# ultravideo/kvazaar

Measured on AMD Instinct MI355X. Metric: CTUs/s (all-intra ultrafast hot path), higher is better.
Workload: dtype u8/i16 (f64 RD costs)

## Files before the change

### kvazaar_amd/csrc/kvz_ctu.hpp

```cpp
#pragma once
#include <type_traits>
#include "../../include/kvz_hip_types.h"
#include "kvz_ops.hpp"
#include "kvz_rdoq.hpp"
#include "kvz_recon.hpp"
#include "kvz_residual.hpp"
#include "kvz_select.hpp"

namespace kvz {

#define KVZ_CTU_THREADS 128
#ifdef KVZ_HOSTSIM
#define KVZ_FOR_THREADS(tid) for (int tid = 0; tid < KVZ_CTU_THREADS; ++tid)
#ifdef KVZ_HOSTSIM_COUNT_SYNCS
static unsigned long long g_kvz_syncs;
#define KVZ_SYNC() (++g_kvz_syncs)
#else
#define KVZ_SYNC()
#endif
#define KVZ_LDS_ADD(p, v) (*(p) += (v))
#else
#define KVZ_FOR_THREADS(tid) for (int tid = (threadIdx.x + lane_rot) & (KVZ_CTU_THREADS - 1), once_ = 1; once_; once_ = 0)
#define KVZ_SYNC() __syncthreads()
#define KVZ_LDS_ADD(p, v) atomicAdd((p), (v))
// ... 27 lines not shown
{
#ifdef KVZ_HOSTSIM
  *dst += v;
#else
  const int x = row16_sum((int)v);
  const u32 total = (u32)(__builtin_amdgcn_readlane(x, 15) + __builtin_amdgcn_readlane(x, 31) + __builtin_amdgcn_readlane(x, 47) + __builtin_amdgcn_readlane(x, 63));
  if ((threadIdx.x & 63) == 0 && total) atomicAdd(dst, total);
#endif
}

#define KVZ_MREF_STRIDE 36
#define KVZ_MREF_ORG 16
#define KVZ_MREF32_STRIDE 68
#define KVZ_MREF32_ORG 32

#ifdef KVZ_HOSTSIM
struct Pk16 { i16 lo, hi; };
KVZ_DEV Pk16 pk_make(int lo, int hi) { Pk16 r = { (i16)lo, (i16)hi }; return r; }
KVZ_DEV Pk16 pk_add(Pk16 a, Pk16 b) { return pk_make(a.lo + b.lo, a.hi + b.hi); }
KVZ_DEV Pk16 pk_sub(Pk16 a, Pk16 b) { return pk_make(a.lo - b.lo, a.hi - b.hi); }
KVZ_DEV u32 pk_absmax(Pk16 a) { return (u32)imax(iabs(a.lo), iabs(a.hi)); }
#else
typedef short Pk16 __attribute__((ext_vector_type(2)));
KVZ_DEV Pk16 pk_make(int lo, int hi) { Pk16 r; r.x = (short)lo; r.y = (short)hi; return r; }
KVZ_DEV Pk16 pk_add(Pk16 a, Pk16 b) { return a + b; }
KVZ_DEV Pk16 pk_sub(Pk16 a, Pk16 b) { return a - b; }
KVZ_DEV u32 pk_absmax(Pk16 a)
{
  const Pk16 m = __builtin_elementwise_max(a, -a);
  return (u32)imax((int)m.x, (int)m.y);
}
KVZ_DEV u32 pk_abs2_biased(Pk16 a, u32 acc)
{
  unsigned x;
  __builtin_memcpy(&x, &a, 4);
  const unsigned t = __builtin_amdgcn_alignbit(x, x, 16);
  Pk16 sw, r;
  __builtin_memcpy(&sw, &t, 4);
  r = a * pk_make(1, -1) + sw;
  unsigned rr;
  __builtin_memcpy(&rr, &r, 4);
  return __builtin_amdgcn_sad_u16(rr, 0x80008000u, acc);
}
#define KVZ_PK_BIAS pk_make(-32768, 0)
#endif

#ifndef KVZ_HOSTSIM
}
#include "kvz_mfma.hpp"
namespace kvz {
#endif

#define KVZ_PROF_PU_AT (2 * KVZ_P_COUNT + 16)
#define KVZ_PROF_WORDS (4 * KVZ_P_COUNT + 16)
enum { KVZ_P_INIT = 0, KVZ_P_REFS, KVZ_P_PRED35, KVZ_P_SATD, KVZ_P_SELECT, KVZ_P_RPRED, KVZ_P_FDCT, KVZ_P_QUANT, KVZ_P_IDCT, KVZ_P_RECON,
       KVZ_P_COST, KVZ_P_COPY, KVZ_P_FINISH, KVZ_P_MISC, KVZ_P_COEFFBITS, KVZ_P_RDOQ, KVZ_P_COUNT };
#if defined(KVZ_CTU_PROFILE) && !defined(KVZ_HOSTSIM)
#define KVZ_PROF(cat) prof_mark(cat)
#define KVZ_PROF_SYNC(cat) do { KVZ_SYNC(); prof_mark(cat); } while (0)
#else
#define KVZ_PROF(cat)
#define KVZ_PROF_SYNC(cat)
#endif

KVZ_DEV u8 load_shared_byte(const u8 *p)
{
#ifdef KVZ_HOSTSIM
  return *p;
#else
  const unsigned long long a = (unsigned long long)p;
  const unsigned w = __hip_atomic_load((const unsigned *)(a & ~3ull), __ATOMIC_RELAXED, __HIP_MEMORY_SCOPE_AGENT);
  return (u8)(w >> (8 * (a & 3)));
#endif
}
KVZ_DEV u32 load_shared_dword(const u8 *p)
{
#ifdef KVZ_HOSTSIM
  u32 w;
  __builtin_memcpy(&w, p, 4);
  return w;
#else
  return __hip_atomic_load((const unsigned *)p, __ATOMIC_RELAXED, __HIP_MEMORY_SCOPE_AGENT);
#endif
}

#ifdef KVZ_HOSTSIM
#define KVZ_ALIGNED(p, n) (p)
#define KVZ_ROLLED
#else
#define KVZ_ALIGNED(p, n) __builtin_assume_aligned((p), (n))
#define KVZ_ROLLED _Pragma("nounroll")
#endif
KVZ_DEV int mover_lane(int tid)
{
#ifndef KVZ_HOSTSIM
  asm volatile("" : "+v"(tid));
#endif
  return tid;
}
template <int N> struct alignas(N) WideBytes { u32 w[N / 4]; };
template <int N> KVZ_DEV WideBytes<N> wide_load(const void *src)
{
  WideBytes<N> v;
  __builtin_memcpy(&v, KVZ_ALIGNED(src, N), N);
  return v;
}
template <int N> KVZ_DEV void wide_store(void *dst, const WideBytes<N> &v) { __builtin_memcpy(KVZ_ALIGNED(dst, N), &v, N); }
// ... 5 lines not shown
  return v;
}

struct CtuCu { u8 type : 1, depth : 2, tr_depth : 3; u8 mode; uint16_t cbf; };

enum { KVZ_CX_SPLIT = KVZ_HIP_CX_SPLIT, KVZ_CX_PART = KVZ_HIP_CX_PART, KVZ_CX_INTRA = KVZ_HIP_CX_INTRA, KVZ_CX_CHROMA = KVZ_HIP_CX_CHROMA,
       KVZ_CX_CBF_LUMA = KVZ_HIP_CX_CBF_LUMA, KVZ_CX_CBF_CHROMA = KVZ_HIP_CX_CBF_CHROMA, KVZ_CX_SYNTAX_COUNT = KVZ_HIP_CX_SIG_CG, KVZ_CX_COUNT = KVZ_HIP_CX_COUNT };
template <bool CABAC> struct CtxSetT { alignas(4) u8 s[CABAC ? 148 : 12]; };

struct CtuModel {
  double lambda, lambda_sqrt;
  uint64_t coeff_weights;
  int qp;
  u8 adaptive, coeff_cabac, no_wpp, search_32x32, rdoq, search_nxn;
  u8 signhide;
  const float *entropy_fbits;
  const u8 *ctx_init;
};
KVZ_HD void ctu_model_from(const kvz_hip_intra_cost_model *src, CtuModel *dst)
{
  dst->lambda = src->lambda; dst->lambda_sqrt = src->lambda_sqrt; dst->coeff_weights = src->coeff_weights; dst->qp = src->qp; dst->adaptive = src->adaptive != 0;
  dst->coeff_cabac = src->coeff_cabac != 0; dst->no_wpp = src->no_wpp != 0; dst->search_32x32 = src->search_32x32 != 0; dst->rdoq = src->rdoq != 0; dst->search_nxn = src->search_nxn != 0;
  dst->signhide = src->signhide != 0;
  dst->entropy_fbits = src->entropy_fbits;
  dst->ctx_init = src->ctx_init;
}
struct CtuModelTable {
  const CtuModel *models = nullptr;
  const uint16_t *model_of_picture = nullptr;
};
KVZ_HD const CtuModel *picture_model(const CtuModelTable &t, long picture) { return t.models + picture_model(t.model_of_picture, picture); }

struct CtuFrames {
  int W, H, wc, hc;
  long frame_px;
  const u8 *src;
  u8 *rec;
  i16 *coeff;
  i16 *coeff_scratch;
  u8 *cu_depth, *cu_mode;
  u8 *cu_part = nullptr;
  u8 *cu_mode4 = nullptr;
  double *ctu_cost;
  unsigned long long *prof;
  u8 *border;
};
#define KVZ_BORDER_BYTES 512

template <bool CABAC> struct CtuSharedT {
  alignas(16) u8 org[1536];
  alignas(16) u8 dec[6144];
#if defined(KVZ_CTU_PROFILE) && !defined(KVZ_HOSTSIM)
  unsigned long long prof_rq[16];
  unsigned long long prof_acc[64];
  int prof_pu;
#endif
  CtuCu cu[4][64];
  u8 ref[3][2][68];
  u8 fref[2][68];
  union {
    struct {
      alignas(16) i16 tb_big[1536];
      alignas(16) u8 c1[1536];
    };
    struct {
      alignas(16) i16 tb_small[2 * 384];
      alignas(8) u8 org_t[256];
      alignas(16) u8 c2[384];
      alignas(16) i16 lv3_coeff[384];
      u8 mref[15][KVZ_MREF_STRIDE];
      u32 satd_raw[35][4];
    };
  };
  alignas(16) i16 lv2_coeff[384];
  alignas(16) i16 lv1_coeff[1536];
#ifdef KVZ_HOSTSIM
  alignas(16) i16 dct32[32 * 32];
#else
  alignas(16) i16 dct_small[64 + 16];
#endif
  u32 acc[16];
  int8_t preds[3];
  int best_mode;
  double cost[4], split_cost[4];
  double res[4];
  double child_bits[4];
  u32 child_acc[4][9];
  int cbf_any;
  u8 bpx_left[3][66];
  u8 bpx_top[3][98];
  uint16_t nb_cu[2][8];
  u8 dcval[3];
  int8_t mode_disp[35];
  int16_t mode_inv[35];
  QuantScalars qs[4][2];
  double mode_bits_cost[3];
  CtxSetT<CABAC> cab, pre[3], post2;
  float entropy_fbits[128];
  u8 ctx_lps[64];
};

using CtuShared = CtuSharedT<true>;
static_assert(__builtin_offsetof(CtuSharedT<true>, fref) == __builtin_offsetof(CtuSharedT<true>, ref) + 408 && __builtin_offsetof(CtuSharedT<false>, fref) == __builtin_offsetof(CtuSharedT<false>, ref) + 408,
              "Tables::mref_tab addresses the filtered references 408 bytes behind the unfiltered ones");
static_assert(KVZ_MREF_STRIDE == kMrefStride && KVZ_MREF_ORG == kMrefOrg && sizeof(((CtuSharedT<true> *)0)->ref[0][0]) == kMrefRefRow && kMrefFiltered == 408,
              "Tables::mref_tab (kvz_tables.hpp) is built for this layout of the reference arrays");
static_assert(KVZ_CTU_THREADS == 128, "two wavefronts per CTU: thread 64 is 'the other wavefront' (recon_cu8, eval_pu, wide_task, rdoq_unit, prices_coeffs, kHookThread), a 16x16 CU's "
                                      "128 (mode, block) pairs are one round of rough_search, plane_sums routes DPP rows per wavefront, and mref_pre[4] covers Tables::mref_tab's 510 entries");

KVZ_HD int plane_off(int c) { return c ? 3072 + (c << 10) : 0; }

struct RdoqLds {
  i32 ptab[2 * 148];
  u8 diag8[64];
  u8 mode4[4][64][4];
  u8 nb_mode4_left[16];
  u8 c4[96];
  alignas(8) i16 lv4_coeff[96];
  u8 pu_mode[4], pu_cbf[4];
  int pu_cbf_c[2];
  int a3x, a3y, n_pu;
  double split_cost3;
  CtxSetT<true> pre3, post3;
};
template <bool CABAC, bool S32 = false, bool RDOQ = false, bool SH = false, bool LISTS = false> struct CtuProgramT {
  static_assert(!(SH && RDOQ), "kvz_rdoq's own sign hiding is not built");
  static_assert(!(LISTS && (RDOQ || SH)), "scaling lists with kvz_rdoq or sign data hiding are not built");
  using CtxSet = CtxSetT<CABAC>;
  const CtuModel *m;
  const Tables *tb;
  CtuFrames F;
  CtuSharedT<CABAC> *s;
  RdoqLds *rl = nullptr;
  const u32 *lf_y = nullptr, *lf_c = nullptr;
  KVZ_DEV ListFactor factor_at(int c, int l2, int e) const { return list_factor(((c ? lf_c : lf_y) + c * KVZ_LIST_PLANE)[list_index(l2, e)]); }
  static constexpr bool NXN = RDOQ;
  KVZ_DEV bool nxn_on() const { return NXN && m->search_nxn; }
  KVZ_DEV bool cabac_on() const { return CABAC && m->coeff_cabac; }
  KVZ_DEV bool hide_on() const { return SH && m->signhide; }
  int frame, cx, cy;
  int a1x, a1y, a2x, a2y;
  static constexpr int kHookThread = 64;
  int a3q = 0;
  int lane_rot = 0;
#if defined(KVZ_CTU_PROFILE) && !defined(KVZ_HOSTSIM)
  unsigned long long t_last;
  __device__ void prof_mark(int cat)
  {
    if (threadIdx.x == 0) {
      const unsigned long long t = __builtin_amdgcn_s_memtime();
      const int at = s->prof_pu ? 32 : 0;
      s->prof_acc[at + cat] += t - t_last;
      s->prof_acc[at + KVZ_P_COUNT + cat] += 1;
      t_last = __builtin_amdgcn_s_memtime();
    }
  }
#endif

  KVZ_DEV static int uni(int v)
  {
#ifdef KVZ_HOSTSIM
    return v;
#else
    return __builtin_amdgcn_readfirstlane(v);
#endif
  }
  KVZ_DEV const u8 *frame_rec(int c) const { return F.rec + (long)frame * F.frame_px + (c == 0 ? 0 : c == 1 ? (long)F.W * F.H : (long)F.W * F.H * 5 / 4); }
  KVZ_DEV const u8 *frame_src(int c) const { return F.src + (long)frame * F.frame_px + (c == 0 ? 0 : c == 1 ? (long)F.W * F.H : (long)F.W * F.H * 5 / 4); }
  KVZ_DEV int ctu_index() const { return (cy >> 6) * F.wc + (cx >> 6); }
  KVZ_DEV i16 *coeff_level(int level) const
  {
    const long ci = (long)frame * F.wc * F.hc + ctu_index();
    return level == 3 ? F.coeff + ci * 6144 : F.coeff_scratch + ci * 6144;
  }
  struct CandView {
    u8 *buf;
    int bias[3], lw[3];
    KVZ_DEV u8 &at(int c, int x, int y) const { return buf[(c == 0 ? bias[0] : (c == 1 ? bias[1] : bias[2])) + (y << (c == 0 ? lw[0] : lw[1])) + x]; }
  };
  KVZ_DEV CandView cand_view(int lv) const
  {
    CandView v;
    if (NXN && lv == 4) {
      v.buf = rl->c4;
      v.lw[0] = 3; v.lw[1] = v.lw[2] = 2;
      v.bias[0] = -(rl->a3y * 8 + rl->a3x);
      v.bias[1] = 64 - ((rl->a3y >> 1) * 4 + (rl->a3x >> 1));
      v.bias[2] = v.bias[1] + 16;
    } else if (lv == 0 || lv == 3) {
      v.buf = s->dec;
      v.lw[0] = 6; v.lw[1] = v.lw[2] = 5;
      v.bias[0] = 0; v.bias[1] = 4096; v.bias[2] = 5120;
    } else if (lv == 1) {
      v.buf = s->c1;
      v.lw[0] = 5; v.lw[1] = v.lw[2] = 4;
      v.bias[0] = -(a1y * 32 + a1x);
      v.bias[1] = 1024 - ((a1y >> 1) * 16 + (a1x >> 1));
      v.bias[2] = v.bias[1] + 256;
    } else {
      v.buf = s->c2;
      v.lw[0] = 4; v.lw[1] = v.lw[2] = 3;
      v.bias[0] = -(a2y * 16 + a2x);
      v.bias[1] = 256 - ((a2y >> 1) * 8 + (a2x >> 1));
      v.bias[2] = v.bias[1] + 64;
// ... 980 lines not shown
        const u32 v = angular_block_satd<true>(log2w, mode, bx, by, xl, yl, t & 1);
        if (!(t & 1)) s->satd_raw[mode][b] = v;
      }
      {
        const int t = KVZ_CTU_THREADS - 1 - tid;
        if (t < 24 * nblk) {
          const int mb = t >> 3, mi = mb >> lb, mode = mi == 0 ? 34 : mi - 1, b = mb & (nblk - 1), bx = (b & ((w >> 3) - 1)) * 8, by = (b >> (log2w - 3)) * 8;
          const u32 v = flat_block_satd8(log2w, mode, bx, by, xl, yl, tid);
          if ((tid & 7) == 0) s->satd_raw[mode][b] = v;
        }
      }
#endif
    }
    }
    KVZ_SYNC();
    KVZ_PROF(KVZ_P_SATD);
    KVZ_FOR_THREADS(tid) {
      const int final_mode = replay_selection(tid, log2w, nblk);
      if (final_mode >= 0) {
        if (tid == 0) s->best_mode = final_mode;
#ifdef KVZ_HOSTSIM
        const int holders = 1;
#else
        const int holders = 64;
#endif
        for (int i = tid; i < (w >> 3) * (w >> 3); i += holders) {
          const int cell = ((yl >> 3) + (i >> (log2w - 3))) * 8 + (xl >> 3) + (i & ((w >> 3) - 1));
          CtuCu *cu = &s->cu[lv][cell];
          cu->type = 1; cu->depth = (u8)depth; cu->mode = (u8)final_mode; cu->tr_depth = (u8)depth;
          set_mode4(lv, cell, final_mode);
        }
      }
    }
    KVZ_SYNC();
    KVZ_PROF(KVZ_P_SELECT);
  }

  struct TuSet { int x, y, lw , lc ; };
  KVZ_DEV static int tu_log2(const TuSet &t, int c) { return c ? t.lc : t.lw; }
  KVZ_DEV i16 *tbuf(const TuSet &t, int p, int c) const
  {
    if (t.lw == 5) return s->tb_big + (c == 0 ? 0 : (c == 1 ? 1024 : 1280));
    return s->tb_small + p * 384 + (c == 0 ? 0 : (c == 1 ? 256 : 320));
  }
  KVZ_DEV int dct_at(int l2, int k, int i) const
  {
#ifdef KVZ_HOSTSIM
    return s->dct32[(k << (10 - l2)) + i];
#else
    return s->dct_small[(l2 == 3 ? 0 : 64) + (k << l2) + i];
#endif
  }

  KVZ_DEV void transform_big(int l2, i16 *x, bool inverse, int tid, int c) const
  {
#ifndef KVZ_HOSTSIM
    if ((tid >> 6) != (c & 1)) return;
    if (l2 == 5) mfma_transform_block<32>(x, x, inverse, tb, tid & 63);
    else mfma_transform_block<16>(x, x, inverse, tb, tid & 63);
#else
    if (tid != 0) return;
    const int n = 1 << l2;
    i16 tmp[32 * 32];
    for (int pass = 0; pass < 2; pass++) {
      const i16 *src = pass == 0 ? x : tmp;
      i16 *dst = pass == 0 ? tmp : x;
      const int shift = inverse ? (pass == 0 ? 7 : 12) : (pass == 0 ? l2 - 1 : l2 + 6);
      for (int e = 0; e < n * n; e++) {
        const int hi = e >> l2, lo = e & (n - 1);
        dst[e] = inverse ? inv_point(n, [&](int k) { return dct_at(l2, k, lo); }, src, hi, n, shift) : fwd_point(n, [&](int i) { return dct_at(l2, hi, i); }, src, lo << l2, shift);
      }
    }
#endif
  }

  enum RowPlan { ROWS_CU8, ROWS_W16, ROWS_W32_Y, ROWS_W32_C };
  KVZ_DEV u32 plane_sums(RowPlan plan, int tid, int c, u32 v, bool packed, int base) const
  {
#ifdef KVZ_HOSTSIM
    (void)tid;
    if (c < 0) return 0;
    if (packed && plan != ROWS_CU8) { s->acc[3 + c] += v & 0xffffffu; s->acc[6 + c] += v >> 24; }
    else s->acc[base + c] += v;
    return 0;
#else
    (void)c;
    if ((plan == ROWS_W16 || plan == ROWS_W32_C) && tid >= 64) return 0;
    const int x = row16_sum((int)v);
    const u32 r0 = (u32)__builtin_amdgcn_readlane(x, 15), r1 = (u32)__builtin_amdgcn_readlane(x, 31), r2 = (u32)__builtin_amdgcn_readlane(x, 47), r3 = (u32)__builtin_amdgcn_readlane(x, 63);
    if (plan == ROWS_CU8) {
      const u32 luma = r0 + r1 + r2 + r3;
      if ((tid & 63) == 0) {
        if (tid < 64) s->acc[base] += luma;
        else { s->acc[base + 1] += r0; s->acc[base + 2] += r1; }
      }
      return tid < 64 ? luma : (tid < 80 ? r0 : r1);
    }
    if ((tid & 63) != 0) return 0;
    auto put = [&](int plane, u32 a, u32 b) {
      if (packed) {
        const u32 ws = (a & 0xffffffu) + (b & 0xffffffu), n = (a >> 24) + (b >> 24);
        if (n) { atomicAdd(&s->acc[3 + plane], ws); atomicAdd(&s->acc[6 + plane], n); }
        else if (ws) atomicAdd(&s->acc[3 + plane], ws);
      } else if (a + b) atomicAdd(&s->acc[base + plane], a + b);
    };
    if (plan == ROWS_W16) { put(0, r0, r1); put(1, r2, 0); put(2, r3, 0); }
    else if (plan == ROWS_W32_Y) { put(0, r0, r1); put(0, r2, r3); }
    else { put(1, r0, r1); put(2, r2, r3); }
    return 0;
#endif
  }
  KVZ_DEV void finish_planes(int lv, int xl, int yl, int depth, int c0, int c1, bool packed) const
  {
    for (int c = c0; c < c1; c++) {
      u32 n = s->acc[6 + c];
      if (packed) { const u32 pk = s->acc[3 + c]; n = pk >> 24; s->acc[3 + c] = pk & 0xffffffu; s->acc[6 + c] = n; }
      if (NXN && lv == 4) { if (c == 0) rl->pu_cbf[rl->n_pu] = n != 0; else rl->pu_cbf_c[c - 1] = n != 0; }
      else {
        CtuCu *cu = &s->cu[lv][(yl >> 3) * 8 + (xl >> 3)];
        cbf_clear(&cu->cbf, depth, c);
        if (n) cbf_set(&cu->cbf, depth, c);
      }
    }
  }
  KVZ_DEV void hide_signs(int tid, int log2y, int log2c, int scan, const i16 *cf_y, i16 *lv_y, const i16 *cf_u, i16 *lv_u, const i16 *cf_v, i16 *lv_v) const
  {
    if constexpr (SH) {
      const int wv = tid >> 6, lane = tid & 63;
      const int c = wv == 0 ? 0 : 1 + (lane >> 4), i = wv == 0 ? lane : (lane & 15), l2 = wv == 0 ? log2y : log2c, groups = 1 << (2 * l2 - 4);
      const bool live = c < 3 && i < groups;
      const i16 *cf = c == 0 ? cf_y : (c == 1 ? cf_u : cf_v);
      i16 *lv = c == 0 ? lv_y : (c == 1 ? lv_u : lv_v);
      auto group_base = [&](int gi) { const int g = scan_group(l2, scan, gi, diag8()); return (((g >> (l2 - 2)) * 4) << l2) + (g & ((1 << (l2 - 2)) - 1)) * 4; };
      auto group_any = [&](int base) {
        unsigned long long acc4 = 0;
        for (int r = 0; r < 4; r++) { unsigned long long four; __builtin_memcpy(&four, lv + base + (r << l2), 8); acc4 |= four; }
        return acc4 != 0;
      };
      const int base = live ? group_base(i) : 0;
      const bool any = live && group_any(base);
#ifdef KVZ_HOSTSIM
      bool first_visited = true;
      for (int j = i + 1; live && j < groups; j++) first_visited = first_visited && !group_any(group_base(j));
#else
      unsigned long long behind = __ballot(any);
      if (wv != 0) behind = (behind >> (16 * ((c - 1) & 1))) & 0xffffull;
      const bool first_visited = ((behind >> i) >> 1) == 0;
#endif
      if (any) {
// ... 157 lines not shown
    *seg = 0;
    if (lw == 4) {
      if (tid < 32) { *seg = tid; return 0; }
      if (tid >= 64 || (tid & 15) >= 8) return -1;
      *seg = tid & 7;
      return tid < 48 ? 1 : 2;
    }
    if (trip == 0) { *seg = tid; return 0; }
    if (tid >= 64) return -1;
    *seg = tid & 31;
    return 1 + (tid >> 5);
  }
  KVZ_DEV void predict_row8(int l2, int mode, int c, int px0, int py, u8 out[8]) const
  {
    const int w = 1 << l2;
    const bool edges = c == 0 && w < 32;
    const u8 *top = s->ref[c][0], *left = s->ref[c][1];
    if (c == 0 && luma_reads_filtered(l2, mode)) { top = s->fref[0]; left = s->fref[1]; }
    if (mode == 0) {
      const int l = left[py + 1], tr = top[w + 1], bl = left[w + 1];
      const int hb = (w - 1) * l + tr + (py + 1) * bl + w, dl = tr - l, wy = w - 1 - py;
      for (int k = 0; k < 8; k++) out[k] = (u8)(((px0 + k) * dl + top[px0 + k + 1] * wy + hb) >> (l2 + 1));
    } else if (mode == 1) {
      const int dc = s->dcval[c];
      for (int k = 0; k < 8; k++) out[k] = (u8)dc;
      if (edges) {
        if (py == 0) for (int k = 0; k < 8; k++) out[k] = (u8)((top[px0 + k + 1] + 3 * dc + 2) >> 2);
        if (px0 == 0) out[0] = (u8)(py == 0 ? (left[1] + 2 * dc + top[1] + 2) >> 2 : (left[py + 1] + 3 * dc + 2) >> 2);
      }
    } else {
      const int disp = s->mode_disp[mode], inv = s->mode_inv[mode];
      const bool vertical = mode >= 18;
      const u8 *main_ref = vertical ? top : left, *side_ref = vertical ? left : top;
      if (vertical) {
        const int delta = (py + 1) * disp, di = delta >> 5, df = delta & 31;
        int r[9];
        if (disp >= 0) for (int j = 0; j < 9; j++) r[j] = main_ref[px0 + di + j + 1];
        else for (int j = 0; j < 9; j++) r[j] = angular_ref(main_ref, side_ref, px0 + di + j, inv);
        for (int k = 0; k < 8; k++) out[k] = (u8)(((32 - df) * r[k] + df * r[k + 1] + 16) >> 5);
        if (edges && mode == 26 && px0 == 0) out[0] = (u8)iclip(0, 255, (int)out[0] + ((left[py + 1] - left[0]) >> 1));
      } else {
        for (int k = 0; k < 8; k++) {
          const int delta = (px0 + k + 1) * disp, di = delta >> 5, df = delta & 31;
          const int r1 = disp >= 0 ? (int)main_ref[py + di + 1] : angular_ref(main_ref, side_ref, py + di, inv);
          const int r2 = disp >= 0 ? (int)main_ref[py + di + 2] : angular_ref(main_ref, side_ref, py + di + 1, inv);
          int v = ((32 - df) * r1 + df * r2 + 16) >> 5;
          if (edges && mode == 10 && py == 0) v = iclip(0, 255, v + ((top[px0 + k + 1] - top[0]) >> 1));
          out[k] = (u8)v;
        }
      }
    }
  }

  KVZ_DEV void recon_tus(int lv, const TuSet &t, int depth, int mode, bool refs_ready = false)
  {
    const int xl = t.x - cx, yl = t.y - cy;
    const CandView cv = cand_view(lv);
    const bool wide = t.lw >= 4;
    if (!refs_ready) build_refs(lv, t.x, t.y, t.lw, t.lc, true, true);
    if (!RDOQ && t.lw == 3) { recon_cu8(lv, t, depth, mode); return; }
#if defined(KVZ_CTU_PROFILE) && !defined(KVZ_HOSTSIM)
    struct InLarge { CtuSharedT<CABAC> *s; bool on; __device__ InLarge(CtuSharedT<CABAC> *s_, bool on_) : s(s_), on(on_) { if (on && threadIdx.x == 0) s->prof_pu = 1; } __device__ ~InLarge() { if (on && threadIdx.x == 0) s->prof_pu = 0; } } in_large(s, !NXN && t.lw >= 4);
#endif
    if (wide) {
      const int umode = uni(mode);
      KVZ_FOR_THREADS(tid) {
        if (tid < 16) s->acc[tid] = 0;
        for (int trip = 0; trip < wide_trips(t.lw); trip++) {
          int seg;
          const int c = wide_task(t.lw, trip, mover_lane(tid), &seg);
          if (c < 0) continue;
          const int l2 = tu_log2(t, c), sh = c ? 1 : 0, py = seg >> (l2 - 3), px0 = (seg << 3) & ((1 << l2) - 1);
          u8 p[8], o[8];
          i16 res[8];
          predict_row8(l2, umode, c, px0, py, p);
          __builtin_memcpy(o, KVZ_ALIGNED(org_at(c, (xl >> sh) + px0, (yl >> sh) + py), 8), 8);
          for (int k = 0; k < 8; k++) res[k] = (i16)((int)o[k] - (int)p[k]);
          __builtin_memcpy(KVZ_ALIGNED(&cv.at(c, (xl >> sh) + px0, (yl >> sh) + py), 8), p, 8);
          __builtin_memcpy(KVZ_ALIGNED(tbuf(t, 0, c) + (seg << 3), 16), res, 16);
        }
      }
    } else
    KVZ_FOR_THREADS(tid) {
      if (tid < 16) s->acc[tid] = 0;
      for (int c = 0; c < 3; c++) {
        const int l2 = tu_log2(t, c), w = 1 << l2, sh = c ? 1 : 0;
        for (int e = tid; e < w * w; e += KVZ_CTU_THREADS) {
          const int px = e & (w - 1), py = e >> l2;
          const u8 p = predict_pixel(l2, mode, c, px, py);
          cv.at(c, (xl >> sh) + px, (yl >> sh) + py) = p;
          tbuf(t, 0, c)[e] = (i16)((int)*org_at(c, (xl >> sh) + px, (yl >> sh) + py) - (int)p);
        }
      }
    }
    KVZ_SYNC();
    KVZ_PROF(KVZ_P_RPRED);
    for (int pass = 0; pass < 2; pass++) {
      KVZ_FOR_THREADS(tid) {
        for (int c = 0; c < 3; c++) {
          const int l2 = tu_log2(t, c), n = 1 << l2;
          const i16 *src = tbuf(t, pass, c);
          i16 *dst = tbuf(t, pass ^ 1, c);
          if (l2 >= 4) {
            if (pass == 0) transform_big(l2, tbuf(t, 0, c), false, tid, c);
            continue;
          }
          for (int e = tid; e < n * n; e += KVZ_CTU_THREADS) {
            const int k = e >> l2, j = e & (n - 1);
            dst[e] = fwd_point(n, [&](int i) { return dct_at(l2, k, i); }, src, j << l2, pass == 0 ? l2 - 1 : l2 + 6);
          }
        }
      }
      KVZ_SYNC();
    }
    KVZ_PROF(KVZ_P_FDCT);
    if (RDOQ && m->rdoq) {
      KVZ_FOR_THREADS(tid) { rdoq_unit(tid, lv, t, true, depth, mode); }
      KVZ_SYNC();
      KVZ_PROF(KVZ_P_RDOQ);
    }
    if (SH && !RDOQ && wide && hide_on()) {
      auto held = [&](int c) { return lv == 0 ? levels_lds(lv, c) : coeff_dst(lv, c, xl, yl); };
      KVZ_FOR_THREADS(tid) {
        for (int trip = 0; trip < wide_trips(t.lw); trip++) {
          int seg;
          const int c = wide_task(t.lw, trip, mover_lane(tid), &seg);
          if (c < 0) continue;
          const QuantScalars q = s->qs[tu_log2(t, c) - 2][c ? 1 : 0];
          i16 cf[8], lvl[8];
          __builtin_memcpy(cf, KVZ_ALIGNED(tbuf(t, 0, c) + (seg << 3), 16), 16);
          for (int k = 0; k < 8; k++) lvl[k] = (i16)quant_level(cf[k], q);
          __builtin_memcpy(KVZ_ALIGNED(held(c) + (seg << 3), 16), lvl, 16);
        }
      }
      KVZ_SYNC();
      KVZ_FOR_THREADS(tid) { hide_signs(tid, t.lw, tu_log2(t, 1), intra_scan_order(mode, depth), tbuf(t, 0, 0), held(0), tbuf(t, 0, 1), held(1), tbuf(t, 0, 2), held(2)); }
      KVZ_SYNC();
      KVZ_FOR_THREADS(tid) {
        const u32 cw_lo = (u32)uni((int)(u32)m->coeff_weights), cw_hi = (u32)uni((int)(u32)(m->coeff_weights >> 32));
        for (int trip = 0; trip < wide_trips(t.lw); trip++) {
          int seg;
          const int c = wide_task(t.lw, trip, mover_lane(tid), &seg);
          u32 packed = 0;
          if (c >= 0) {
            const QuantScalars q = s->qs[tu_log2(t, c) - 2][c ? 1 : 0];
            i16 lvl[8], dq[8];
            __builtin_memcpy(lvl, KVZ_ALIGNED(held(c) + (seg << 3), 16), 16);
            u32 wsum = 0, nz = 0;
            for (int k = 0; k < 8; k++) {
              const LevelCost lc = level_cost(lvl[k], cw_lo, cw_hi);
              wsum += lc.weight;
              nz += lc.nonzero;
              dq[k] = dequant_level(lvl[k], q);
            }
            packed = wsum | (nz << 24);
            if (lv == 0) __builtin_memcpy(KVZ_ALIGNED(coeff_dst(lv, c, xl, yl) + (seg << 3), 16), lvl, 16);
            __builtin_memcpy(KVZ_ALIGNED(tbuf(t, 1, c) + (seg << 3), 16), dq, 16);
// ... 19 lines not shown
              ListFactor f{ 0, 0 };
              if constexpr (LISTS) f = factor_at(c, l2, (seg << 3) + k);
              const int level = LISTS ? quant_level(cf[k], q, f.fwd) : quant_level(cf[k], q);
              lvl[k] = (i16)level;
              const LevelCost lc = level_cost(level, cw_lo, cw_hi);
              wsum += lc.weight;
              nz += lc.nonzero;
              dq[k] = LISTS ? dequant_level(level, q, f.inv) : dequant_level(level, q);
            }
            packed = wsum | (nz << 24);
            __builtin_memcpy(KVZ_ALIGNED(coeff_dst(lv, c, xl, yl) + (seg << 3), 16), lvl, 16);
            if (to_stage) __builtin_memcpy(KVZ_ALIGNED(levels_lds(lv, c) + (seg << 3), 16), lvl, 16);
            __builtin_memcpy(KVZ_ALIGNED(tbuf(t, 1, c) + (seg << 3), 16), dq, 16);
          }
          plane_sums(wide_rows(t.lw, trip), tid, c, packed, true, 3);
        }
      }
    } else
    KVZ_FOR_THREADS(tid) {
      for (int c = 0; c < 3; c++) {
        const int l2 = tu_log2(t, c), n2 = 1 << (2 * l2);
        const QuantScalars q = s->qs[l2 - 2][c ? 1 : 0];
        i16 *cout = coeff_dst(lv, c, xl, yl);
        i16 *stage = (cabac_on() && lv == 0) ? levels_lds(lv, c) : nullptr;
        const i16 *src = tbuf(t, 0, c);
        i16 *dq = tbuf(t, 1, c);
        u32 wsum = 0, nz = 0;
        for (int e = tid; e < n2; e += KVZ_CTU_THREADS) {
          int level;
          if (RDOQ && m->rdoq) { level = (stage ? stage : cout)[e]; if (stage) cout[e] = (i16)level; }
          else if constexpr (LISTS) { level = quant_level(src[e], q, factor_at(c, l2, e).fwd); cout[e] = (i16)level; }
          else { level = quant_level(src[e], q); cout[e] = (i16)level; }
          if (stage && !(RDOQ && m->rdoq)) stage[e] = (i16)level;
          const LevelCost lc = level_cost(level, m->coeff_weights);
          wsum += lc.weight;
          nz += lc.nonzero;
          if constexpr (LISTS) dq[e] = dequant_level(level, q, factor_at(c, l2, e).inv);
          else dq[e] = dequant_level(level, q);
        }
        block_add(&s->acc[3 + c], wsum);
        block_add(&s->acc[6 + c], nz);
      }
    }
    KVZ_SYNC();
    KVZ_PROF(KVZ_P_QUANT);
    for (int pass = 0; pass < 2; pass++) {
      KVZ_FOR_THREADS(tid) {
        for (int c = 0; c < 3; c++) {
          const int l2 = tu_log2(t, c), n = 1 << l2;
          if (!s->acc[6 + c]) continue;
          const i16 *src = tbuf(t, pass ^ 1, c);
          i16 *dst = tbuf(t, pass, c);
          if (l2 >= 4) {
            if (pass == 0) transform_big(l2, tbuf(t, 1, c), true, tid, c);
            continue;
          }
          for (int e = tid; e < n * n; e += KVZ_CTU_THREADS) {
            const int j = e >> l2, i = e & (n - 1);
            dst[e] = inv_point(n, [&](int k) { return dct_at(l2, k, i); }, src, j, n, pass == 0 ? 7 : 12);
          }
        }
      }
      KVZ_SYNC();
    }
    KVZ_PROF(KVZ_P_IDCT);
    KVZ_FOR_THREADS(tid) {
      if (wide) {
        for (int trip = 0; trip < wide_trips(t.lw); trip++) {
          int seg;
          const int c = wide_task(t.lw, trip, mover_lane(tid), &seg);
          u32 ssd = 0;
          if (c >= 0) {
            const int l2 = tu_log2(t, c), sh = c ? 1 : 0, py = seg >> (l2 - 3), px0 = (seg << 3) & ((1 << l2) - 1);
            u8 *rp = &cv.at(c, (xl >> sh) + px0, (yl >> sh) + py);
            u8 v[8], o[8];
            __builtin_memcpy(v, KVZ_ALIGNED(rp, 8), 8);
            __builtin_memcpy(o, KVZ_ALIGNED(org_at(c, (xl >> sh) + px0, (yl >> sh) + py), 8), 8);
            if (s->acc[6 + c] != 0) {
              i16 res[8];
              __builtin_memcpy(res, KVZ_ALIGNED(tbuf(t, 1, c) + (seg << 3), 16), 16);
              for (int k = 0; k < 8; k++) v[k] = (u8)recon_sample(v[k], res[k]);
              __builtin_memcpy(KVZ_ALIGNED(rp, 8), v, 8);
            }
            for (int k = 0; k < 8; k++) ssd += sq_err(o[k], v[k]);
          }
          plane_sums(wide_rows(t.lw, trip), tid, c, ssd, false, 0);
        }
      } else
      for (int c = 0; c < 3; c++) {
        const int l2 = tu_log2(t, c), w = 1 << l2, sh = c ? 1 : 0;
        const bool has = s->acc[6 + c] != 0;
        u32 ssd = 0;
        for (int e = tid; e < w * w; e += KVZ_CTU_THREADS) {
          u8 *rp = &cv.at(c, (xl >> sh) + (e & (w - 1)), (yl >> sh) + (e >> l2));
          int v = *rp;
          if (has) { v = recon_sample(v, tbuf(t, 1, c)[e]); *rp = (u8)v; }
          ssd += sq_err(*org_at(c, (xl >> sh) + (e & (w - 1)), (yl >> sh) + (e >> l2)), v);
        }
        block_add(&s->acc[c], ssd);
      }
      if (tid == 0) finish_planes(lv, xl, yl, depth, 0, 3, false);
    }
    KVZ_SYNC();
    KVZ_PROF(KVZ_P_RECON);
  }

#ifdef KVZ_HOSTSIM
// ... 947 lines not shown
          }
        } else
        eval_cu(3, qx, qy, 3, &s->cost[3], &s->cbf_any, [&](int tid) { if (tid == kHookThread) { cu_header(3, qx - cx, qy - cy, 3); price_modes(); } }, [&](int tid) { if (tid == 0) s->split_cost[2] += s->cost[3]; });
      }
    }
    const bool split_wins2 = s->split_cost[2] < s->cost[2];
    if (split_wins2) {
      commit(3, 2, 2, -1, false, xl, yl, 16, 2, true);
    } else {
      commit(2, 3, 3, 2, true, xl, yl, 16, 2, false);
    }
  }

  KVZ_DEV void search_d1(int x1, int y1)
  {
    const int xl = x1 - cx, yl = y1 - cy;
    const bool inside = x1 + 32 <= F.W && y1 + 32 <= F.H;
    int *cbf1 = reinterpret_cast<int *>(&s->child_acc[0][0]);
    auto d1_first = [&](int tid) { if (tid == 0) { *cbf1 = 0; price_modes(); } };
    auto d1_last = [&](int tid) {
      ctx_swap_lanes(&s->cab, &s->pre[1], tid);
      if (tid == 0) {
        double sc = split_flag_cost(1, x1, y1, 1);
        if (inside && !*cbf1) sc = 2147483647;
        s->split_cost[1] = sc;
      }
    };
    if (inside) eval_cu(1, x1, y1, 1, &s->cost[1], cbf1, d1_first, d1_last);
    else {
      KVZ_FOR_THREADS(tid) { d1_first(tid); d1_last(tid); }
      KVZ_SYNC();
    }
    const bool descend = !inside || *cbf1;
    if (!descend) return;
    u8 *stash = reinterpret_cast<u8 *>(coeff_level(0));
    if (inside) {
      KVZ_FOR_THREADS(tid) { copy_run(stash, s->c1, 1536, tid); }
      KVZ_SYNC();
    }
    for (int q2 = 0; q2 < 4; q2++) {
      if (!(s->split_cost[1] < s->cost[1])) break;
      search_d2(x1 + (q2 & 1) * 16, y1 + (q2 >> 1) * 16);
    }
    if (inside && !(s->split_cost[1] < s->cost[1])) {
      KVZ_SYNC();
      KVZ_FOR_THREADS(tid) { copy_run(s->c1, stash, 1536, tid); }
      KVZ_SYNC();
    }
  }

  KVZ_DEV void run()
  {
#if defined(KVZ_CTU_PROFILE) && !defined(KVZ_HOSTSIM)
    if (threadIdx.x == 0) { for (int i = 0; i < 64; i++) s->prof_acc[i] = 0; for (int i = 0; i < 16; i++) s->prof_rq[i] = 0; s->prof_pu = 0; }
    t_last = __builtin_amdgcn_s_memtime();
#endif
    init();
    if constexpr (RDOQ) {
      KVZ_FOR_THREADS(tid) {
        if (m->rdoq) for (int v = tid; v < 2 * KVZ_CX_COUNT; v += KVZ_CTU_THREADS) rl->ptab[v] = (i32)(s->entropy_fbits[s->pre[0].s[v >> 1] ^ (v & 1)] * 32768.0f);
        if (tid < 64) rl->diag8[tid] = tb->diag8[tid];
      }
      KVZ_SYNC();
    }
    KVZ_PROF(KVZ_P_INIT);
    KVZ_FOR_THREADS(tid) {
      if (tid == 0) { cu_header(0, 0, 0, 0); s->cost[0] = 1.7e+308; s->split_cost[0] = split_flag_cost(0, cx, cy, 0); }
    }
    KVZ_SYNC();
    for (int q1 = 0; q1 < 4; q1++) {
      const int x1 = cx + (q1 & 1) * 32, y1 = cy + (q1 >> 1) * 32;
      if (x1 >= F.W || y1 >= F.H) continue;
      a1x = x1 - cx; a1y = y1 - cy;
      const bool search32 = S32 && m->search_32x32;
      load_org([&](int tid) {
        ctx_copy_lanes(&s->pre[1], &s->cab, tid);
        if (tid == 0) { cu_header(1, x1 - cx, y1 - cy, 1); s->cost[1] = 1.7e+308; if (!search32) s->split_cost[1] = split_flag_cost(1, x1, y1, 1); }
      });
      if (search32) search_d1(x1, y1);
      else {
        for (int q2 = 0; q2 < 4; q2++) search_d2(x1 + (q2 & 1) * 16, y1 + (q2 >> 1) * 16);
        if (x1 + 32 <= F.W && y1 + 32 <= F.H) try_merge(x1, y1, 1);
      }
      const bool split_wins1 = s->split_cost[1] < s->cost[1];
      if (split_wins1) commit(2, 1, 1, -1, false, x1 - cx, y1 - cy, 32, 1, true);
      else commit(1, 2, 3, 1, true, x1 - cx, y1 - cy, 32, 1, false);
    }
    bool attempt0 = false;
    if (cx + 64 <= F.W && cy + 64 <= F.H) { const CtuCu d1 = s->cu[1][0]; attempt0 = d1.type == 1 && d1.depth == 1; }
    if (attempt0) { write_rec(); try_merge(cx, cy, 0); }
    const bool split_wins0 = s->split_cost[0] < s->cost[0];
    if (split_wins0) {
      commit(1, 0, 0, -1, false, 0, 0, 64, 0, true);
      if (!attempt0) write_rec();
    } else {
      commit(0, 0, -1, -1, true, 0, 0, 64, 0, false);
      write_rec();
    }
    KVZ_PROF(KVZ_P_MISC);
    if (m->adaptive && cabac_on()) { code_ctu_residual(); KVZ_PROF_SYNC(KVZ_P_PRED35); }
    finish_info();
    KVZ_PROF(KVZ_P_FINISH);
#if defined(KVZ_CTU_PROFILE) && !defined(KVZ_HOSTSIM)
    __syncthreads();
    if (threadIdx.x == 0) {
      for (int i = 0; i < 2 * KVZ_P_COUNT; i++) { atomicAdd(&F.prof[i], s->prof_acc[i]); atomicAdd(&F.prof[KVZ_PROF_PU_AT + i], s->prof_acc[32 + i]); }
      for (int i = 0; i < 16; i++) atomicAdd(&F.prof[2 * KVZ_P_COUNT + i], s->prof_rq[i]);
    }
#endif
  }
};
using CtuProgram = CtuProgramT<true>;

}
```

Before: 3.063 million.

## Add specialized fused 16x16 CU reconstruction and paired chroma MFMA transforms for 32x32 TUs

Adds a dedicated recon_cu16 path for non-RDOQ 16x16 luma TUs with 8x8 chroma. Wave 0 runs luma prediction, the MFMA transform, quantisation and reconstruction, while wave 1 handles both chroma planes with the per-lane 8x8 matrix routines. The stages use wave-level syncs and per-lane coded flags instead of block-wide barriers and LDS accumulators. For 32x32 TUs, the two 16x16 chroma transforms are batched into one paired MFMA call on a single wave. The profiling buffers also gain a separate 32x32 bucket. The risks are extra code size and register pressure, plus subtle correctness around the coded flags and which wave owns which plane.

```diff
diff --git a/kvazaar_amd/csrc/kvz_ctu.hpp b/kvazaar_amd/csrc/kvz_ctu.hpp
--- a/kvazaar_amd/csrc/kvz_ctu.hpp
+++ b/kvazaar_amd/csrc/kvz_ctu.hpp
@@ -103,7 +103,8 @@
 #endif
 
 #define KVZ_PROF_PU_AT (2 * KVZ_P_COUNT + 16)
-#define KVZ_PROF_WORDS (4 * KVZ_P_COUNT + 16)
+#define KVZ_PROF_W32_AT (4 * KVZ_P_COUNT + 16)
+#define KVZ_PROF_WORDS (6 * KVZ_P_COUNT + 16)
 enum { KVZ_P_INIT = 0, KVZ_P_REFS, KVZ_P_PRED35, KVZ_P_SATD, KVZ_P_SELECT, KVZ_P_RPRED, KVZ_P_FDCT, KVZ_P_QUANT, KVZ_P_IDCT, KVZ_P_RECON,
        KVZ_P_COST, KVZ_P_COPY, KVZ_P_FINISH, KVZ_P_MISC, KVZ_P_COEFFBITS, KVZ_P_RDOQ, KVZ_P_COUNT };
 #if defined(KVZ_CTU_PROFILE) && !defined(KVZ_HOSTSIM)
@@ -215,7 +216,7 @@
   alignas(16) u8 dec[6144];
 #if defined(KVZ_CTU_PROFILE) && !defined(KVZ_HOSTSIM)
   unsigned long long prof_rq[16];
-  unsigned long long prof_acc[64];
+  unsigned long long prof_acc[96];
   int prof_pu;
 #endif
   CtuCu cu[4][64];
@@ -312,7 +313,7 @@
   {
     if (threadIdx.x == 0) {
       const unsigned long long t = __builtin_amdgcn_s_memtime();
-      const int at = s->prof_pu ? 32 : 0;
+      const int at = 32 * s->prof_pu;
       s->prof_acc[at + cat] += t - t_last;
       s->prof_acc[at + KVZ_P_COUNT + cat] += 1;
       t_last = __builtin_amdgcn_s_memtime();
@@ -1399,13 +1400,15 @@
 #endif
   }
 
-  KVZ_DEV void transform_big(int l2, i16 *x, bool inverse, int tid, int c) const
+  KVZ_DEV void transform_big(int l2, i16 *x, bool inverse, int tid, int c, bool pair = false) const
   {
 #ifndef KVZ_HOSTSIM
-    if ((tid >> 6) != (c & 1)) return;
+    if ((tid >> 6) != (c ? 1 : 0)) return;
     if (l2 == 5) mfma_transform_block<32>(x, x, inverse, tb, tid & 63);
+    else if (pair) mfma_transform_blocks16<2>(x, x, inverse, tb, tid & 63);
     else mfma_transform_block<16>(x, x, inverse, tb, tid & 63);
 #else
+    (void)pair;
     if (tid != 0) return;
     const int n = 1 << l2;
     i16 tmp[32 * 32];
@@ -1421,7 +1424,13 @@
 #endif
   }
 
-  enum RowPlan { ROWS_CU8, ROWS_W16, ROWS_W32_Y, ROWS_W32_C };
+#ifdef KVZ_HOSTSIM
+  KVZ_DEV static bool big_pairs(const TuSet &) { return false; }
+#else
+  KVZ_DEV static bool big_pairs(const TuSet &t) { return t.lw == 5; }
+#endif
+
+  enum RowPlan { ROWS_CU8, ROWS_CU16, ROWS_W16, ROWS_W32_Y, ROWS_W32_C };
   KVZ_DEV u32 plane_sums(RowPlan plan, int tid, int c, u32 v, bool packed, int base) const
   {
 #ifdef KVZ_HOSTSIM
@@ -1431,7 +1440,6 @@
     else s->acc[base + c] += v;
     return 0;
 #else
-    (void)c;
     if ((plan == ROWS_W16 || plan == ROWS_W32_C) && tid >= 64) return 0;
     const int x = row16_sum((int)v);
     const u32 r0 = (u32)__builtin_amdgcn_readlane(x, 15), r1 = (u32)__builtin_amdgcn_readlane(x, 31), r2 = (u32)__builtin_amdgcn_readlane(x, 47), r3 = (u32)__builtin_amdgcn_readlane(x, 63);
@@ -1442,6 +1450,15 @@
         else { s->acc[base + 1] += r0; s->acc[base + 2] += r1; }
       }
       return tid < 64 ? luma : (tid < 80 ? r0 : r1);
+    }
+    if (plan == ROWS_CU16) {
+      u32 a = r0 + r1 + r2 + r3, n = 0;
+      if (packed) { a = (r0 & 0xffffffu) + (r1 & 0xffffffu) + (r2 & 0xffffffu) + (r3 & 0xffffffu); n = (r0 >> 24) + (r1 >> 24) + (r2 >> 24) + (r3 >> 24); }
+      if ((tid & 63) == 0) {
+        if (packed) { s->acc[3 + c] = a; s->acc[6 + c] = n; }
+        else s->acc[base + c] = a;
+      }
+      return packed ? n : a;
     }
     if ((tid & 63) != 0) return 0;
     auto put = [&](int plane, u32 a, u32 b) {
@@ -1705,6 +1722,177 @@
     }
   }
 
+  KVZ_DEV void predict_chroma_pair(int l2, int mode, int x, int y, u8 *pu, u8 *pv) const
+  {
+    const u8 *top_u = s->ref[1][0], *left_u = s->ref[1][1], *top_v = s->ref[2][0], *left_v = s->ref[2][1];
+    if (mode == 0) { *pu = planar_pixel(l2, x, y, top_u, left_u); *pv = planar_pixel(l2, x, y, top_v, left_v); return; }
+    if (mode == 1) { *pu = s->dcval[1]; *pv = s->dcval[2]; return; }
+    const bool vertical = mode >= 18;
+    const int px = vertical ? x : y, py = vertical ? y : x;
+    const int delta_pos = (py + 1) * s->mode_disp[mode], di = delta_pos >> 5, df = delta_pos & 31, inv = s->mode_inv[mode];
+    const int i1 = px + di, i2 = i1 + 1;
+    const bool main1 = i1 >= -1, main2 = i2 >= -1;
+    const int o1 = main1 ? i1 + 1 : (128 + (-1 - i1) * inv) >> 8, o2 = main2 ? i2 + 1 : (128 + (-1 - i2) * inv) >> 8;
+    auto plane = [&](const u8 *top, const u8 *left) {
+      const u8 *main_ref = vertical ? top : left, *side_ref = vertical ? left : top;
+      const int r1 = (main1 ? main_ref : side_ref)[o1], r2 = (main2 ? main_ref : side_ref)[o2];
+      return (u8)(((32 - df) * r1 + df * r2 + 16) >> 5);
+    };
+    *pu = plane(top_u, left_u);
+    *pv = plane(top_v, left_v);
+  }
+
+  KVZ_DEV void recon_cu16(int lv, const TuSet &t, int depth, int mode)
+  {
+    const int xl = t.x - cx, yl = t.y - cy, xc = xl >> 1, yc = yl >> 1;
+    const CandView cv = cand_view(lv);
+    const int umode = uni(mode);
+    const bool to_stage = cabac_on() && lv == 0;
+    KVZ_LANE_VAR(WideBytes<16>, mat_f);
+    KVZ_LANE_VAR(WideBytes<16>, mat_i);
+    KVZ_LANE_VAR(u32, pred_org);
+    KVZ_LANE_VAR(u32, coded);
+#ifdef KVZ_HOSTSIM
+#define KVZ_CU16_CODED(tid, c) ((void)KVZ_LANE(coded, tid), s->acc[6 + (c)] != 0)
+#else
+#define KVZ_CU16_CODED(tid, c) (((KVZ_LANE(coded, tid) >> ((c) == 2 ? 1 : 0)) & 1u) != 0)
+#endif
+    KVZ_FOR_THREADS(tid) {
+      if (tid < 3) s->acc[3 * tid] = 0;
+      if (tid >= 64 && tid < 70) s->acc[1 + (tid - 64) + ((tid - 64) >> 1)] = 0;
+      if (tid < 32) {
+        const int seg = mover_lane(tid), py = seg >> 1, px0 = (seg << 3) & 15;
+        u8 p[8], o[8];
+        i16 res[8];
+        predict_row8(4, umode, 0, px0, py, p);
+        __builtin_memcpy(o, KVZ_ALIGNED(org_at(0, xl + px0, yl + py), 8), 8);
+        for (int k = 0; k < 8; k++) res[k] = (i16)((int)o[k] - (int)p[k]);
+        __builtin_memcpy(KVZ_ALIGNED(&cv.at(0, xl + px0, yl + py), 8), p, 8);
+        __builtin_memcpy(KVZ_ALIGNED(tbuf(t, 0, 0) + (seg << 3), 16), res, 16);
+      } else if (tid >= 64) {
+        const int e = tid - 64, px = e & 7, py = e >> 3;
+        cu8_matrix_rows<3>(tb, e, KVZ_LANE(mat_f, tid), KVZ_LANE(mat_i, tid));
+        u8 pu, pv;
+        predict_chroma_pair(3, umode, px, py, &pu, &pv);
+        cv.at(1, xc + px, yc + py) = pu;
+        cv.at(2, xc + px, yc + py) = pv;
+        const u8 ou = *org_at(1, xc + px, yc + py), ov = *org_at(2, xc + px, yc + py);
+        KVZ_LANE(pred_org, tid) = (u32)pu | ((u32)ou << 8) | ((u32)pv << 16) | ((u32)ov << 24);
+        tbuf(t, 0, 1)[e] = (i16)((int)ou - (int)pu);
+        tbuf(t, 0, 2)[e] = (i16)((int)ov - (int)pv);
+      }
+    }
+    KVZ_WAVE_SYNC();
+    KVZ_PROF(KVZ_P_RPRED);
+    KVZ_FOR_THREADS(tid) {
+      if (tid < 64) transform_big(4, tbuf(t, 0, 0), false, tid, 0);
+      else {
+        const int e = tid - 64;
+        tbuf(t, 1, 1)[e] = cu8_fwd_first<3>(tbuf(t, 0, 1), e, KVZ_LANE(mat_f, tid));
+        tbuf(t, 1, 2)[e] = cu8_fwd_first<3>(tbuf(t, 0, 2), e, KVZ_LANE(mat_f, tid));
+      }
+    }
+    KVZ_WAVE_SYNC();
+    KVZ_PROF(KVZ_P_FDCT);
+    KVZ_FOR_THREADS(tid) {
+      const u32 cw_lo = (u32)uni((int)(u32)m->coeff_weights), cw_hi = (u32)uni((int)(u32)(m->coeff_weights >> 32));
+      if (tid < 64) {
+        u32 packed = 0;
+        if (tid < 32) {
+          const int seg = mover_lane(tid);
+          const QuantScalars q = s->qs[2][0];
+          i16 cf[8], lvl[8], dq[8];
+          __builtin_memcpy(cf, KVZ_ALIGNED(tbuf(t, 0, 0) + (seg << 3), 16), 16);
+          u32 wsum = 0, nz = 0;
+          for (int k = 0; k < 8; k++) {
+            ListFactor f{ 0, 0 };
+            if constexpr (LISTS) f = factor_at(0, 4, (seg << 3) + k);
+            const int level = LISTS ? quant_level(cf[k], q, f.fwd) : quant_level(cf[k], q);
+            lvl[k] = (i16)level;
+            const LevelCost lc = level_cost(level, cw_lo, cw_hi);
+            wsum += lc.weight;
+            nz += lc.nonzero;
+            dq[k] = LISTS ? dequant_level(level, q, f.inv) : dequant_level(level, q);
+          }
+          packed = wsum | (nz << 24);
+          __builtin_memcpy(KVZ_ALIGNED(coeff_dst(lv, 0, xl, yl) + (seg << 3), 16), lvl, 16);
+          if (to_stage) __builtin_memcpy(KVZ_ALIGNED(levels_lds(lv, 0) + (seg << 3), 16), lvl, 16);
+          __builtin_memcpy(KVZ_ALIGNED(tbuf(t, 1, 0) + (seg << 3), 16), dq, 16);
+        }
+        KVZ_LANE(coded, tid) = plane_sums(ROWS_CU16, tid, tid < 32 ? 0 : -1, packed, true, 3) != 0;
+      } else {
+        const int e = tid - 64;
+        const QuantScalars q = s->qs[1][1];
+        auto plane = [&](int c) {
+          const int cf = cu8_fwd_second<3>(tbuf(t, 1, c), e, KVZ_LANE(mat_f, tid));
+          ListFactor f{ 0, 0 };
+          if constexpr (LISTS) f = factor_at(c, 3, e);
+          const int level = LISTS ? quant_level(cf, q, f.fwd) : quant_level(cf, q);
+          coeff_dst(lv, c, xl, yl)[e] = (i16)level;
+          if (to_stage) levels_lds(lv, c)[e] = (i16)level;
+          tbuf(t, 0, c)[cu8_transposed<3>(e)] = LISTS ? dequant_level(level, q, f.inv) : dequant_level(level, q);
+          return level_cost(level, cw_lo, cw_hi).word();
+        };
+        const u32 wu = plane(1), wv = plane(2);
+        const u32 nu = plane_sums(ROWS_CU16, tid, 1, wu, true, 3), nv = plane_sums(ROWS_CU16, tid, 2, wv, true, 3);
+        KVZ_LANE(coded, tid) = (u32)(nu != 0) | ((u32)(nv != 0) << 1);
+      }
+    }
+    KVZ_WAVE_SYNC();
+    KVZ_PROF(KVZ_P_QUANT);
+    KVZ_FOR_THREADS(tid) {
+      if (tid < 64) { if (uni((int)KVZ_CU16_CODED(tid, 0))) transform_big(4, tbuf(t, 1, 0), true, tid, 0); }
+      else {
+        const int e = tid - 64;
+        if (KVZ_CU16_CODED(tid, 1)) tbuf(t, 1, 1)[cu8_transposed<3>(e)] = cu8_inv_first<3>(tbuf(t, 0, 1), e, KVZ_LANE(mat_i, tid));
+        if (KVZ_CU16_CODED(tid, 2)) tbuf(t, 1, 2)[cu8_transposed<3>(e)] = cu8_inv_first<3>(tbuf(t, 0, 2), e, KVZ_LANE(mat_i, tid));
+      }
+    }
+    KVZ_WAVE_SYNC();
+    KVZ_PROF(KVZ_P_IDCT);
+    KVZ_FOR_THREADS(tid) {
+      if (tid < 64) {
+        u32 ssd = 0;
+        if (tid < 32) {
+          const int seg = mover_lane(tid), py = seg >> 1, px0 = (seg << 3) & 15;
+          u8 *rp = &cv.at(0, xl + px0, yl + py);
+          u8 v[8], o[8];
+          __builtin_memcpy(v, KVZ_ALIGNED(rp, 8), 8);
+          __builtin_memcpy(o, KVZ_ALIGNED(org_at(0, xl + px0, yl + py), 8), 8);
+          if (KVZ_CU16_CODED(tid, 0)) {
+            i16 res[8];
+            __builtin_memcpy(res, KVZ_ALIGNED(tbuf(t, 1, 0) + (seg << 3), 16), 16);
+            for (int k = 0; k < 8; k++) v[k] = (u8)recon_sample(v[k], res[k]);
+            __builtin_memcpy(KVZ_ALIGNED(rp, 8), v, 8);
+          }
+          for (int k = 0; k < 8; k++) ssd += sq_err(o[k], v[k]);
+        }
+        plane_sums(ROWS_CU16, tid, tid < 32 ? 0 : -1, ssd, false, 0);
+      } else {
+        const int e = tid - 64, px = e & 7, py = e >> 3;
+        auto plane = [&](int c) {
+          const u32 po = KVZ_LANE(pred_org, tid) >> (c == 2 ? 16 : 0);
+          int v = (int)(po & 0xffu);
+          if (KVZ_CU16_CODED(tid, c)) {
+            v = recon_sample(v, cu8_inv_second<3>(tbuf(t, 1, c), e, KVZ_LANE(mat_i, tid)));
+            cv.at(c, xc + px, yc + py) = (u8)v;
+          }
+          return sq_err((int)((po >> 8) & 0xffu), v);
+        };
+        const u32 su = plane(1), sv = plane(2);
+        plane_sums(ROWS_CU16, tid, 1, su, false, 0);
+        plane_sums(ROWS_CU16, tid, 2, sv, false, 0);
+      }
+    }
+#undef KVZ_CU16_CODED
+    KVZ_SYNC();
+    KVZ_FOR_THREADS(tid) {
+      if (tid == 0) finish_planes(lv, xl, yl, depth, 0, 3, false);
+    }
+    if (cabac_on()) KVZ_SYNC();
+    KVZ_PROF(KVZ_P_RECON);
+  }
+
   KVZ_DEV void recon_tus(int lv, const TuSet &t, int depth, int mode, bool refs_ready = false)
   {
     const int xl = t.x - cx, yl = t.y - cy;
@@ -1713,8 +1901,9 @@
     if (!refs_ready) build_refs(lv, t.x, t.y, t.lw, t.lc, true, true);
     if (!RDOQ && t.lw == 3) { recon_cu8(lv, t, depth, mode); return; }
 #if defined(KVZ_CTU_PROFILE) && !defined(KVZ_HOSTSIM)
-    struct InLarge { CtuSharedT<CABAC> *s; bool on; __device__ InLarge(CtuSharedT<CABAC> *s_, bool on_) : s(s_), on(on_) { if (on && threadIdx.x == 0) s->prof_pu = 1; } __device__ ~InLarge() { if (on && threadIdx.x == 0) s->prof_pu = 0; } } in_large(s, !NXN && t.lw >= 4);
-#endif
+    struct InLarge { CtuSharedT<CABAC> *s; int on; __device__ InLarge(CtuSharedT<CABAC> *s_, int on_) : s(s_), on(on_) { if (on && threadIdx.x == 0) s->prof_pu = on; } __device__ ~InLarge() { if (on && threadIdx.x == 0) s->prof_pu = 0; } } in_large(s, (!NXN && t.lw >= 4) ? t.lw - 3 : 0);
+#endif
+    if (!RDOQ && t.lw == 4 && t.lc == 3 && !hide_on()) { recon_cu16(lv, t, depth, mode); return; }
     if (wide) {
       const int umode = uni(mode);
       KVZ_FOR_THREADS(tid) {
@@ -1755,7 +1944,7 @@
           const i16 *src = tbuf(t, pass, c);
           i16 *dst = tbuf(t, pass ^ 1, c);
           if (l2 >= 4) {
-            if (pass == 0) transform_big(l2, tbuf(t, 0, c), false, tid, c);
+            if (pass == 0 && !(big_pairs(t) && c == 2)) transform_big(l2, tbuf(t, 0, c), false, tid, c, big_pairs(t) && c == 1);
             continue;
           }
           for (int e = tid; e < n * n; e += KVZ_CTU_THREADS) {
@@ -1881,7 +2070,7 @@
           const i16 *src = tbuf(t, pass ^ 1, c);
           i16 *dst = tbuf(t, pass, c);
           if (l2 >= 4) {
-            if (pass == 0) transform_big(l2, tbuf(t, 1, c), true, tid, c);
+            if (pass == 0 && !(big_pairs(t) && c == 2 && s->acc[7])) transform_big(l2, tbuf(t, 1, c), true, tid, c, big_pairs(t) && c == 1 && s->acc[8]);
             continue;
           }
           for (int e = tid; e < n * n; e += KVZ_CTU_THREADS) {
@@ -2935,7 +3124,7 @@
   KVZ_DEV void run()
   {
 #if defined(KVZ_CTU_PROFILE) && !defined(KVZ_HOSTSIM)
-    if (threadIdx.x == 0) { for (int i = 0; i < 64; i++) s->prof_acc[i] = 0; for (int i = 0; i < 16; i++) s->prof_rq[i] = 0; s->prof_pu = 0; }
+    if (threadIdx.x == 0) { for (int i = 0; i < 96; i++) s->prof_acc[i] = 0; for (int i = 0; i < 16; i++) s->prof_rq[i] = 0; s->prof_pu = 0; }
     t_last = __builtin_amdgcn_s_memtime();
 #endif
     init();
@@ -2987,7 +3176,7 @@
 #if defined(KVZ_CTU_PROFILE) && !defined(KVZ_HOSTSIM)
     __syncthreads();
     if (threadIdx.x == 0) {
-      for (int i = 0; i < 2 * KVZ_P_COUNT; i++) { atomicAdd(&F.prof[i], s->prof_acc[i]); atomicAdd(&F.prof[KVZ_PROF_PU_AT + i], s->prof_acc[32 + i]); }
+      for (int i = 0; i < 2 * KVZ_P_COUNT; i++) { atomicAdd(&F.prof[i], s->prof_acc[i]); atomicAdd(&F.prof[KVZ_PROF_PU_AT + i], s->prof_acc[32 + i]); atomicAdd(&F.prof[KVZ_PROF_W32_AT + i], s->prof_acc[64 + i]); }
       for (int i = 0; i < 16; i++) atomicAdd(&F.prof[2 * KVZ_P_COUNT + i], s->prof_rq[i]);
     }
 #endif
```

Result: faster. 3.181 million (median of 6 runs) (+3.8%).
